# torchmd/torchmd-net

Hardware: AMD Instinct MI355X
Metric: molecules/sec (64-atom molecules) TensorNet E+F (higher is better)
Workload: dtype f32; 1 GPU; BASELINE configs[1]: TensorNet F=128 L=2 K=32 rc=5.0, S-mol64 256 molecules x 64 atoms per GPU, energies + forces, random-init weights (seed 0); atoms_per_gpu=16384, pairs_per_gpu=193709, directed_edges_per_gpu=403802, parallelism=molecule-sharded x1, RCCL all-reduce of energies, rank_step=eager: tmdnet_build_graph (pair-count read-back) + tmdnet_energy_forces

## Files before the change

### torchmd-net_amd/csrc/tn_api.hip

```cpp
#include <hip/hip_runtime.h>

#include <algorithm>
#include <cmath>
#include <cstdio>
#include <cstdlib>
#include <cstring>
#include <map>
#include <unordered_map>
#include <string>
#include <vector>

#include "tn_chain.h"
#include "tn_heads.h"
#include "tn_model.h"
#include "tn_tlin9.h"
#include "tn_small.h"
#include "tn_interp.h"
#include "tn_virial.h"

using namespace tn;

static const char* kCatNames[CAT_COUNT] = {"graph", "gemm_edge", "gemm_node", "message", "pair_bwd", "embed_scatter", "elementwise", "edge_table"};

int fail(tmdnet_model* m, int code, const std::string& msg) {
  if (m) m->err = msg;
  return code;
}
thread_local tmdnet_model* g_cur = nullptr;
thread_local int g_gemm_cat = CAT_GEMM_NODE;
thread_local const int* g_mdev = nullptr;
thread_local int g_madd = 0;
thread_local const uint16_t* g_wsb_debug = nullptr;

void gemm(hipStream_t s, const float* A, int64_t lda, const float* W, int64_t ldw, const float* bias, float* C, int64_t ldc, int M,
          int N, int K, int flags, float* pre, int64_t ldpre, const float* aux, int64_t ldaux,
          const float* rowscale) {
  GemmArgs a{};
  a.A = A;
  a.W[0] = W;
  a.C = C;
  a.bias[0] = bias;
  a.pre = pre;
  a.aux = aux;
  a.rowscale = rowscale;
  a.lda = lda;
// ... 183 lines not shown
  g.counts = c.take<int>(8);
  g.mstart = c.take<int>(B);
  g.mend = c.take<int>(B);
  g.nlow = c.take<int>(N);
  g.ntot = c.take<int>(N);
  g.rowptr = c.take<int>(N + 1);
  g.pairptr = c.take<int>(N + 1);
  g.col = c.take<int>(ecap);
  g.epair = c.take<int>(ecap);
  g.esign = c.take<float>(ecap);
  g.pair_i = c.take<int>(pcap);
  g.pair_j = c.take<int>(pcap);
  g.pd = c.take<float>(pcap + 1);
  g.pdelta = c.take<float>(pcap * 3);
  g.prhat = c.take<float>(pcap * 3);
  g.ecap = ecap;
  g.pcap = pcap;
  g.perm = c.take<int>(N);
  g.iota = c.take<int>(N);
  g.cell_key = c.take<int>(N);
  g.cell_key_sorted = c.take<int>(N);
  g.cell_start = c.take<int>(8 * N + 2);
  g.pos_s = c.take<float>(3 * N);
  g.z_s = c.take<int64_t>(N);
  g.boxd = c.take<float>(12);
  g.cgrid = c.take<int>(4);
  g.bat_s = c.take<int>(N);
  g.bat_c = c.take<int64_t>(N);
  g.z_c = c.take<int64_t>(N);
  g.tix = c.take<int>(N);
  g.tz = c.take<int>(64);
  g.sort_tmp_bytes = cell_sort_temp_bytes(N);
  g.sort_tmp = c.take<char>((int64_t)g.sort_tmp_bytes);
  if (total) *total = c.off;
  return g;
}

namespace {
bool cell_applicable(const tmdnet_model* m, int64_t n_atoms, int64_t n_mol, int box_mode) {
  const int* n = m->cell_n;
  if (n_mol < 1 || box_mode == 2 || n_atoms < 1) return false;
  if (n[0] < 0) return true;
  if (n[0] < 1 || n[1] < 1 || n[2] < 1) return false;
  return (int64_t)n[0] * n[1] * n[2] <= 8 * n_atoms;
}
void set_cell(Graph& g, const tmdnet_model* m, bool on, int64_t n_mol = 1) {
  g.use_cell = on ? (n_mol > 1 ? 2 : 1) : 0;
  const bool explicit_grid = m->cell_n[0] > 0;
  g.ncx = explicit_grid ? m->cell_n[0] : 0;
  g.ncy = explicit_grid ? m->cell_n[1] : 0;
  g.ncz = explicit_grid ? m->cell_n[2] : 0;
}

}
int rb_ntp(const tmdnet_model* m, int64_t n_atoms, int64_t n_pairs) {
  if (!m->rb_fwd || m->et || m->train || n_pairs < 0 || n_atoms < m->rb_min_atoms) return 0;
  return embed_rb_ntp(m->last_nt);
}
namespace {

FwdBuffers carve_fwd(void* ws, const tmdnet_hparams& hp, int64_t N, int64_t B, int64_t P, bool bwd, size_t* total, int ntp = 0,
                     int lean = 0) {
  Carver c(ws);
  FwdBuffers b{};
  const int64_t F = hp.hidden_channels, K = hp.num_rbf, L = hp.num_layers, Z = hp.max_z, H = hp.head_hidden;
  const int64_t P1 = P + 1, N9 = N * 9 * F;
// ... 782 lines not shown
  for (const auto& j : m->image_jobs) {
    if (j.fm) launch_split_weight_fm(m->dev + j.src_off, j.n, j.k, m->dev_sb + j.dst_off, s);
    else launch_split_weight_tiles(m->dev + j.src_off, j.n, j.k, m->dev_sb + j.dst_off, s);
  }
  const int F = m->hp.hidden_channels;
  launch_ztables(m->P.emb, m->P.emb2_waT, m->P.emb2_wbT, m->P.emb2_b, m->hp.max_z, F, const_cast<float*>(m->P.Utab),
                 const_cast<float*>(m->P.Vtab), s);
  m->tabs_pending = true;
  if (m->rb_fwd)
    launch_embed_rb_images(m->P.Wdp, m->P.bdp, F, m->hp.num_rbf, m->rb_img, m->rb_img + embed_rb_image_elems(F, m->hp.num_rbf, false), s);
  HIP_TRY(m, hipGetLastError());
  return TMDNET_OK;
}

int tmdnet_set_option(tmdnet_model* m, const char* name, double value) {
  if (!m || !name) return TMDNET_ERR_INVALID;
  const std::string n(name);
  if (n == "edge_table_min_pairs") {
    m->tab_min_pairs = value < 0 ? 0 : (int64_t)value;
    return TMDNET_OK;
  }
  if (n == "embed_rb_min_atoms") {
    m->rb_min_atoms = value < 0 ? 0 : (int64_t)value;
    return TMDNET_OK;
  }
  if (n == "chain_min_atoms") {
    m->chain_min_atoms = value < 0 ? 0 : (value > 9e18 ? INT64_MAX : (int64_t)value);
    return TMDNET_OK;
  }
  if (n == "chain_mask") {
    m->chain_mask = (int)value & 7;
    return TMDNET_OK;
  }
  if (n == "pair_rows_bf16") {
    if (!m->et) return fail(m, TMDNET_ERR_INVALID, "pair_rows_bf16 applies to the Equivariant Transformer handle only");
    m->pair_bf16 = value == 2.0 ? 2 : (value != 0.0 ? 1 : 0);
    return TMDNET_OK;
  }
  if (n == "recompute_pair_rows") {
    if (m->et || m->tn2) return fail(m, TMDNET_ERR_INVALID, "recompute_pair_rows applies to the TensorNet handle only");
    m->recompute_rows = value != 0.0;
    return TMDNET_OK;
  }
  return fail(m, TMDNET_ERR_INVALID, "unknown option: " + n);
}

int tmdnet_get_info(const tmdnet_model* m, const char* name, double* value) {
  if (!m || !name || !value) return TMDNET_ERR_INVALID;
  const std::string n(name);
  if (m->tabs_pending && n.rfind("edge_table_", 0) == 0 && n != "edge_table_min_pairs")
    if (const int rc = ensure_radial_tables(const_cast<tmdnet_model*>(m), nullptr)) return rc;
  if (n == "edge_table_T") *value = m->tabs.ok ? m->tabs.T : 0;
  else if (n == "edge_table_err_value") *value = m->tabs.err_value;
  else if (n == "edge_table_err_slope") *value = m->tabs.err_slope;
  else if (n == "edge_table_min_pairs") *value = (double)m->tab_min_pairs;
  else if (n == "pair_rows_bf16") *value = (double)m->pair_bf16;
  else if (n == "embed_rb_min_atoms") *value = (double)m->rb_min_atoms;
  else if (n == "chain_min_atoms") *value = (double)m->chain_min_atoms;
  else if (n == "chain_mask") *value = (double)m->chain_mask;
  else if (n == "chain_last") *value = (double)m->chain_last;
  else if (n == "recompute_pair_rows") *value = m->recompute_rows ? 1.0 : 0.0;
  else if (n == "embed_rb") *value = m->rb_fwd ? 1.0 : 0.0;
  else if (n == "species_last_build") *value = (double)m->last_nt;
  else if (n == "halo_active_first") *value = (double)m->halo_active[0];
  else if (n == "halo_active_rows") *value = (double)m->halo_active[1];
  else if (n == "message_route_last") *value = (double)m->msg_route_last[0];
  else if (n == "message_adjoint_route_last") *value = (double)m->msg_route_last[1];
  else return TMDNET_ERR_INVALID;
  return TMDNET_OK;
}

int tmdnet_set_cell_grid(tmdnet_model* m, int32_t ncx, int32_t ncy, int32_t ncz) {
  if (!m) return TMDNET_ERR_INVALID;
  if (ncx < 0 || ncy < 0 || ncz < 0) ncx = ncy = ncz = -1;
  m->cell_n[0] = ncx;
  m->cell_n[1] = ncy;
  m->cell_n[2] = ncz;
  return TMDNET_OK;
}

int tmdnet_graph_workspace_bytes(const tmdnet_model* m, int64_t n_atoms, int64_t n_mol, size_t* bytes) {
  if (!m || !bytes || n_atoms < 0 || n_mol < 0) return TMDNET_ERR_INVALID;
  const int64_t ecap = (int64_t)m->hp.max_num_neighbors * n_atoms;
  carve_graph(nullptr, n_atoms, n_mol, ecap, bytes);
  return TMDNET_OK;
}

int tmdnet_build_graph(tmdnet_model* m, void* stream, void* graph_ws, size_t graph_ws_bytes, int64_t n_atoms, int64_t n_mol,
                       const float* pos, const int64_t* batch, const int64_t* z, const float* box, int32_t box_mode,
                       int64_t counts_host[8]) {
  if (!m || !graph_ws || !counts_host || n_atoms < 0 || n_mol < 0) return TMDNET_ERR_INVALID;
  if (n_atoms >= (int64_t)1 << 30) return fail(m, TMDNET_ERR_INVALID, "n_atoms too large for 32-bit indices");
  hipStream_t s = reinterpret_cast<hipStream_t>(stream);
  const int64_t ecap = (int64_t)m->hp.max_num_neighbors * n_atoms;
  size_t need = 0;
  Graph g = carve_graph(graph_ws, n_atoms, n_mol, ecap, &need);
  if (need > graph_ws_bytes) return fail(m, TMDNET_ERR_WORKSPACE, "graph workspace too small");
  if (box_mode != 0 && !box) return fail(m, TMDNET_ERR_INVALID, "box_mode != 0 needs a box");
  const bool cell = cell_applicable(m, n_atoms, n_mol, box_mode);
  set_cell(g, m, cell, n_mol);
  if (cell && m->halo_fn && m->atom_w && !m->et && !m->tn2) g.ghost_w = m->atom_w;
  m->graph_no_ghost_pairs = g.ghost_w != nullptr;
  m->graph_is_cell = cell;
  m->graph_cell_multi = cell && n_mol > 1;
  m->graph_has_z = z != nullptr;
  m->g_pos = pos;
  m->g_box = box;
  m->g_box_mode = box_mode;
  CurScope cur_(m);
  {
    ProfScope ps_(s, CAT_GRAPH, 0.0, (double)n_atoms * 20);
    if (cell) {
      launch_fill(reinterpret_cast<float*>(g.counts), 0.f, 8, s);
      launch_cell_phase1(g, pos, batch, box_mode == 1 ? box : nullptr, (int)n_atoms, m->hp.cutoff_lower, m->hp.cutoff_upper, true, s,
                         (int)n_mol);
      launch_scan_counts(g, (int)n_atoms, s);
    } else {
      launch_graph_build_phase1(g, pos, batch, box, box_mode, (int)n_atoms, (int)n_mol, m->hp.cutoff_lower, m->hp.cutoff_upper,
                                true, s);
    }
    if (z) launch_prepare_z(g, z, cell ? g.perm : nullptr, (int)n_atoms, m->hp.max_z, s);
    if (z && m->rb_fwd && n_atoms >= m->rb_min_atoms) launch_type_map(g, (int)n_atoms, m->hp.max_z, s);
  }
  int counts[8] = {0, 0, 0, 0, 0, 0, 0, 0};
  HIP_TRY(m, hipMemcpyAsync(counts, g.counts, sizeof(counts), hipMemcpyDeviceToHost, s));
  HIP_TRY(m, hipStreamSynchronize(s));
  for (int k = 0; k < 8; ++k) counts_host[k] = counts[k];
  m->last_nt = (z && m->rb_fwd && n_atoms >= m->rb_min_atoms) ? counts[6] : 0;
  m->lastE = counts[1];
  remember_graph(m, graph_ws);
  if (counts[5])
    return fail(m, TMDNET_ERR_INVALID, "batch index out of range: every entry must be in [0, " + std::to_string(n_mol) + ")");
  if (counts[4])
    return fail(m, TMDNET_ERR_INVALID, "atomic number out of range: every z must be in [0, max_z = " + std::to_string(m->hp.max_z) + ")");
  if (counts[2])
    return fail(m, TMDNET_ERR_OVERFLOW, "Found num_pairs > max_num_pairs, please increase max_num_pairs (found " +
                                            std::to_string(counts[1]) + " edges, capacity " + std::to_string(ecap) + ")");
  m->lastE = counts[1];
  {
    ProfScope ps_(s, CAT_GRAPH, 0.0, (double)counts[1] * 12 + (double)counts[0] * 40);
    if (cell) {
      launch_cell_phase2(g, (int)n_atoms, m->hp.cutoff_lower, m->hp.cutoff_upper, true, s);
      launch_nbr_link_wave(g, (int)n_atoms, s);
    } else {
      launch_graph_build_phase2(g, pos, batch, box, box_mode, (int)n_atoms, (int)n_mol, m->hp.cutoff_lower, m->hp.cutoff_upper, true,
                                s);
    }
  }
  HIP_TRY(m, hipGetLastError());
  return TMDNET_OK;
}

int tmdnet_build_graph_static(tmdnet_model* m, void* stream, void* graph_ws, size_t graph_ws_bytes, int64_t n_atoms, int64_t n_mol,
                              const float* pos, const int64_t* batch, const int64_t* z, const float* box, int32_t box_mode) {
  if (!m || !graph_ws || n_atoms < 0 || n_mol < 0) return TMDNET_ERR_INVALID;
  hipStream_t s = reinterpret_cast<hipStream_t>(stream);
  const int64_t ecap = (int64_t)m->hp.max_num_neighbors * n_atoms;
  size_t need = 0;
  Graph g = carve_graph(graph_ws, n_atoms, n_mol, ecap, &need);
  if (need > graph_ws_bytes) return fail(m, TMDNET_ERR_WORKSPACE, "graph workspace too small");
  if (box_mode != 0 && !box) return fail(m, TMDNET_ERR_INVALID, "box_mode != 0 needs a box");
  const bool cell = cell_applicable(m, n_atoms, n_mol, box_mode);
  set_cell(g, m, cell, n_mol);
  m->graph_no_ghost_pairs = false;
  m->graph_is_cell = cell;
  m->graph_cell_multi = cell && n_mol > 1;
  m->graph_has_z = z != nullptr;
  m->g_pos = pos;
  m->g_box = box;
  m->g_box_mode = box_mode;
  CurScope cur_(m);
  {
    ProfScope ps_(s, CAT_GRAPH, 0.0, (double)n_atoms * 20);
    if (cell) {
      launch_fill(reinterpret_cast<float*>(g.counts), 0.f, 8, s);
      launch_cell_phase1(g, pos, batch, box_mode == 1 ? box : nullptr, (int)n_atoms, m->hp.cutoff_lower, m->hp.cutoff_upper, true, s,
// ... 826 lines not shown
  }
  m->prof.on = false;
  m->prof.recs.clear();
  m->prof.used = 0;
  return TMDNET_OK;
}

int tmdnet_profile_end_records(tmdnet_model* m, void* stream, int64_t cap, int32_t* cat, double* ms, double* flops, double* bytes,
                               char* labels, int64_t* n_out) {
  if (!m || !cat || !ms || !flops || !bytes || !n_out || cap < 0) return TMDNET_ERR_INVALID;
  HIP_TRY(m, hipStreamSynchronize(reinterpret_cast<hipStream_t>(stream)));
  int64_t n = 0;
  for (const ProfRec& r : m->prof.recs) {
    if (n >= cap) break;
    float t = 0.f;
    HIP_TRY(m, hipEventElapsedTime(&t, r.a, r.b));
    cat[n] = r.cat;
    ms[n] = t;
    flops[n] = r.flops;
    bytes[n] = r.bytes;
    if (labels) std::memcpy(labels + 64 * n, r.label, 64);
    ++n;
  }
  *n_out = (int64_t)m->prof.recs.size();
  m->prof.on = false;
  m->prof.recs.clear();
  m->prof.used = 0;
  return TMDNET_OK;
}

int tmdnet_profile_num_categories(void) { return CAT_COUNT; }
const char* tmdnet_profile_category_name(int idx) { return idx >= 0 && idx < CAT_COUNT ? kCatNames[idx] : nullptr; }

int tmdnet_debug_tensor(tmdnet_model* m, void* stream, const char* name, float* out, int64_t numel) {
  if (m && m->et) return et_debug_tensor(m, reinterpret_cast<hipStream_t>(stream), name, out, numel);
  if (!m || !name || !out || !m->has_last) return TMDNET_ERR_STATE;
  hipStream_t s = reinterpret_cast<hipStream_t>(stream);
  const int64_t F = m->hp.hidden_channels, K = m->hp.num_rbf, N = m->lastN, P1 = m->lastP + 1;
  const FwdBuffers& b = m->last;
  const float* src = nullptr;
  int64_t n = 0;
  std::string nm(name);
  if (nm == "X_embed") { src = b.X[0]; n = N * 9 * F; }
  else if (nm.rfind("X_layer", 0) == 0) {
    int l = std::atoi(nm.c_str() + 7);
    if (l < 0 || l >= m->hp.num_layers) return TMDNET_ERR_INVALID;
    src = b.X[l + 1]; n = N * 9 * F;
  }
  else if (nm.rfind("Pn", 0) == 0 || nm.rfind("Mi", 0) == 0 || (nm.rfind("D", 0) == 0 && nm.size() == 2)) {
    const int l = std::atoi(nm.c_str() + (nm[0] == 'D' ? 1 : 2));
    if (l < 0 || l >= m->hp.num_layers) return TMDNET_ERR_INVALID;
    src = nm[0] == 'P' ? b.Pn[l] : (nm[0] == 'M' ? b.Mi[l] : b.D[l]);
    n = N * 9 * F;
  }
  else if (nm == "x") { src = b.x; n = N * F; }
  else if (nm == "phi") { src = b.phi; n = P1 * K; }
  else if (nm == "Q") { src = b.Q; n = P1 * 3 * F; }
  else if (nm == "u0") { src = b.u0; n = N * 9 * F; }
  else if (nm == "G_embed") { src = b.G; n = N * 9 * F; }
  else if (nm == "charges" && m->tn2) { src = m->tn2_last_chg; n = N * (int64_t)(m->hp.num_layers + 1) * m->tn2->hp.q_dim; }
  else return fail(m, TMDNET_ERR_INVALID, "unknown debug tensor");
  if (!src || numel != n) return fail(m, TMDNET_ERR_INVALID, "debug tensor size mismatch: expected " + std::to_string(n));
  HIP_TRY(m, hipMemcpyAsync(out, src, sizeof(float) * n, hipMemcpyDeviceToDevice, s));
  return TMDNET_OK;
}

int tmdnet_debug_gemm_dual(void* stream, const float* A, const float* A2, const float* W, const float* bias, float* C, float* C2,
// ... 207 lines not shown
```

### torchmd-net_amd/csrc/tn_graph_wave.hip

```cpp
#include <cstdlib>

#include "tn_common.h"
#include "tn_kernels.h"

namespace tn {

static inline int cdivw(int64_t a, int64_t b) { return (int)((a + b - 1) / b); }

__device__ __forceinline__ float pair_d2(const float* __restrict__ pos, int hi, int lo, const float* __restrict__ box, float& dx,
                                         float& dy, float& dz) {
  return pair_geometry(pos, hi, lo, box, dx, dy, dz);
}

template <bool FILL>
__device__ __forceinline__ void nbr_wave_row(const Graph& g, const float* __restrict__ pos, const int64_t* __restrict__ batch,
                                             const float* __restrict__ box, int box_mode, int N, int B, float lo2, float up2, int loop,
                                             int i, int lane) {
  int64_t b = batch[i];
  int j0 = 0, j1 = N;
  if (b < 0 || b >= B) {
    b = 0;
    j1 = 0;
  } else if (!g.counts[3]) {
    j0 = g.mstart[b];
    j1 = g.mend[b];
  }
  const float* bx = box_mode == 0 ? nullptr : (box_mode == 1 ? box : box + b * 9);
  const int P = FILL ? g.counts[0] : 0;
  int e = FILL ? g.rowptr[i] : 0, p = FILL ? g.pairptr[i] : 0;
  int nl = 0, nt = 0;
  const unsigned long long lt = lane == 0 ? 0ull : (~0ull >> (64 - lane));
  for (int base = j0; base < j1; base += 64) {
    const int j = base + lane;
    bool hit = false, self = false;
    float dx = 0.f, dy = 0.f, dz = 0.f, d2 = 0.f;
// ... 40 lines not shown
  }
  if (!FILL && lane == 0) {
    g.nlow[i] = nl;
    g.ntot[i] = nt;
  }
  if (FILL && i == 0 && lane == 0) g.pd[P] = 0.f;
}

template <bool FILL>
__global__ __launch_bounds__(256) void k_nbr_wave(Graph g, const float* __restrict__ pos, const int64_t* __restrict__ batch,
                                                  const float* __restrict__ box, int box_mode, int N, int B, float lo2, float up2,
                                                  int loop) {
  const int i = blockIdx.x * 4 + (threadIdx.x >> 6);
  const int lane = threadIdx.x & 63;
  if (i >= N) return;
  if (FILL && g.counts[2]) return;
  nbr_wave_row<FILL>(g, pos, batch, box, box_mode, N, B, lo2, up2, loop, i, lane);
}

__device__ __forceinline__ void nbr_link_row(const Graph& g, int i, int lane) {
  const int e0 = g.rowptr[i], e1 = g.rowptr[i + 1];
  for (int e = e0 + lane; e < e1; e += 64) {
    const int j = g.col[e];
    if (j <= i) continue;
    int lo = g.rowptr[j], hi = lo + g.nlow[j] - 1;
    const int base = lo;
    while (lo < hi) {
      const int mid = (lo + hi) >> 1;
      if (g.col[mid] < i) lo = mid + 1; else hi = mid;
    }
    g.epair[e] = g.pairptr[j] + (lo - base);
  }
}
__global__ __launch_bounds__(256) void k_nbr_link_wave(Graph g, int N) {
  const int i = blockIdx.x * 4 + (threadIdx.x >> 6);
  const int lane = threadIdx.x & 63;
  if (i >= N || g.counts[2]) return;
  nbr_link_row(g, i, lane);
}

constexpr int GS_MAX_ATOMS = 256;
constexpr int GS_ECAP = 16384;
__global__ __launch_bounds__(1024) void k_graph_small(Graph g, const float* __restrict__ pos, const int64_t* __restrict__ batch,
                                                      const float* __restrict__ box, int box_mode, int N, int B, float lo2, float up2,
                                                      int loop, const int64_t* __restrict__ z, int max_z) {
  __shared__ int s_mstart[GS_MAX_ATOMS], s_mend[GS_MAX_ATOMS], s_nlow[GS_MAX_ATOMS], s_ntot[GS_MAX_ATOMS];
  __shared__ int s_rowptr[GS_MAX_ATOMS + 1], s_pairptr[GS_MAX_ATOMS + 1], s_counts[8], c_low[4], c_tot[4];
  __shared__ float s_pos[3 * GS_MAX_ATOMS];
  __shared__ int64_t s_batch[GS_MAX_ATOMS];
  __shared__ int s_col[GS_ECAP];
  const bool col_lds = g.ecap <= GS_ECAP;
  const int tid = threadIdx.x, lane = tid & 63, wave = tid >> 6;
  const bool mol_lds = B <= GS_MAX_ATOMS;
  Graph gl = g;
  gl.nlow = s_nlow;
  gl.ntot = s_ntot;
  gl.rowptr = s_rowptr;
  gl.pairptr = s_pairptr;
  gl.counts = s_counts;
  if (mol_lds) {
    gl.mstart = s_mstart;
    gl.mend = s_mend;
  }
  if (col_lds) gl.col = s_col;
  for (int k = tid; k < 3 * N; k += 1024) s_pos[k] = pos[k];
  if (tid < N) s_batch[tid] = batch[tid];
  for (int i = tid; i < B; i += 1024) gl.mstart[i] = gl.mend[i] = 0;
  if (tid < 8) s_counts[tid] = 0;
  __syncthreads();
  if (tid < N) {
// ... 66 lines not shown
  if (!s_counts[2]) {
    for (int i = wave; i < N; i += 16) nbr_wave_row<true>(gl, s_pos, s_batch, box, box_mode, N, B, lo2, up2, loop, i, lane);
    __syncthreads();
    for (int i = wave; i < N; i += 16) nbr_link_row(gl, i, lane);
    if (col_lds) {
      __syncthreads();
      const int E = s_counts[1];
      for (int e = tid; e < E; e += 1024) g.col[e] = s_col[e];
    }
  }
  if (tid <= N) {
    g.rowptr[tid] = s_rowptr[tid];
    g.pairptr[tid] = s_pairptr[tid];
  }
  if (tid < N) {
    g.nlow[tid] = s_nlow[tid];
    g.ntot[tid] = s_ntot[tid];
  }
  if (mol_lds && tid < B) {
    g.mstart[tid] = s_mstart[tid];
    g.mend[tid] = s_mend[tid];
  }
  if (tid < 8) g.counts[tid] = s_counts[tid];
}
bool graph_small_ok(int N) {
  static const bool off = getenv("TMDNET_NO_GRAPH_SMALL") != nullptr;
  return !off && N > 0 && N <= GS_MAX_ATOMS;
}
void launch_graph_small(const Graph& g, const float* pos, const int64_t* batch, const float* box, int box_mode, int N, int B, float lo,
                        float up, bool loop, const int64_t* z, int max_z, hipStream_t s) {
  hipLaunchKernelGGL(k_graph_small, dim3(1), dim3(1024), 0, s, g, pos, batch, box, box_mode, N, B, lo * lo, up * up, (int)loop, z, max_z);
}

void launch_nbr_count_wave(const Graph& g, const float* pos, const int64_t* batch, const float* box, int box_mode, int N, int B,
                           float lo, float up, bool loop, hipStream_t s) {
  hipLaunchKernelGGL(k_nbr_wave<false>, dim3(cdivw(N, 4)), dim3(256), 0, s, g, pos, batch, box, box_mode, N, B, lo * lo, up * up,
                     (int)loop);
}
void launch_nbr_fill_link_wave(const Graph& g, const float* pos, const int64_t* batch, const float* box, int box_mode, int N, int B,
                               float lo, float up, bool loop, hipStream_t s) {
  hipLaunchKernelGGL(k_nbr_wave<true>, dim3(cdivw(N, 4)), dim3(256), 0, s, g, pos, batch, box, box_mode, N, B, lo * lo, up * up,
                     (int)loop);
  hipLaunchKernelGGL(k_nbr_link_wave, dim3(cdivw(N, 4)), dim3(256), 0, s, g, N);
}
void launch_nbr_link_wave(const Graph& g, int N, hipStream_t s) {
  hipLaunchKernelGGL(k_nbr_link_wave, dim3(cdivw(N, 4)), dim3(256), 0, s, g, N);
}

}
```

### torchmd-net_amd/csrc/tn_kernels.h

```cpp
#pragma once
#include <hip/hip_runtime.h>
#include <stdint.h>

namespace tn {

struct Graph {
  int* mstart;
  int* mend;
  int* nlow;
  int* ntot;
  int* rowptr;
  int* pairptr;
  int* col;
  int* epair;
  float* esign;
  int* pair_i;
  int* pair_j;
  float* pd;
  float* pdelta;
  float* prhat;
  int* counts;
  int* tix;
  int* tz;
  int64_t ecap, pcap;
  int* perm;
  int* iota;
  int* cell_key;
  int* cell_key_sorted;
  int* cell_start;
  float* pos_s;
  int64_t* z_s;
  float* boxd;
  int* cgrid;
  int* bat_s;
  int64_t* bat_c;
  int64_t* z_c;
  void* sort_tmp;
  size_t sort_tmp_bytes;
  int ncx, ncy, ncz;
  int use_cell;
  const float* ghost_w;
  int max_z;
  int small_mols;
};

struct RadialParams {
  const float* means;
  const float* betas;
  int K;
  float lo, up;
};

void launch_graph_build_phase1(const Graph& g, const float* pos, const int64_t* batch, const float* box, int box_mode, int N,
                               int B, float lo, float up, bool loop, hipStream_t s);
void launch_graph_build_phase2(const Graph& g, const float* pos, const int64_t* batch, const float* box, int box_mode, int N,
                               int B, float lo, float up, bool loop, hipStream_t s);
void launch_export_pairs(const Graph& g, int N, bool include_transpose, bool loop, int64_t max_pairs, const int* perm,
                         int64_t* neighbors, float* deltas, float* distances, int* num_pairs, hipStream_t s);

void launch_neighbor_grad(const int64_t* nb, const float* deltas, const float* dist, const float* g_delta, const float* g_dist,
                          int64_t M, int N, float* out, hipStream_t s);

void launch_radial(const Graph& g, int P, RadialParams rp, float* phi, float* dphi, float* C, float* dC, hipStream_t s);

void launch_ztables(const float* emb, const float* WaT, const float* WbT, const float* b2, int Z, int F, float* Utab, float* Vtab,
                    hipStream_t s);
void launch_embed_scatter(const Graph& g, int N, int F, const int64_t* z, const float* Utab, const float* Vtab, const float* Q,
                          const float* C, float* u0, float* s0n, hipStream_t s);
void launch_layernorm_fwd(const float* x, const float* w, const float* b, int rows, int R, float* y, float* xhat, float* rstd,
                          hipStream_t s);
void launch_layernorm_bwd(const float* g, const float* xhat, const float* rstd, const float* w, int rows, int R, float* gx,
                          hipStream_t s);
void launch_norm_x(const float* X, float* Xh, int N, int F, hipStream_t s);
struct PairRowTable;
enum MsgRoute {
  MSG_NONE = 0,
// ... 51 lines not shown

void launch_head_bwd(const float* ao, const float* O2, int N, int H, float std, float* g_ao, hipStream_t s);
void launch_readout_bwd(const float* X, const float* g_feat, int N, int F, float* G, hipStream_t s);
void launch_update_bwd(const float* G, const float* D, const float* q, const int64_t* batch, int N, int F, float* gD,
                       hipStream_t s);
void launch_message_bwd_node(const float* gCh, const float* Pn, const float* Mi, const float* q, const int64_t* batch, int o3, int N,
                             int F, float* gMi, float* gPn, hipStream_t s);
void launch_norm_bwd(const float* X, const float* gXh_lin, int N, int F, float* G, hipStream_t s);
void launch_norm_bwd_update_bwd(const float* X, const float* gXh_lin, int N, int F, float* G, const float* Dn, const float* q,
                                const int64_t* batch, float* gD, hipStream_t s);
void launch_norm_bwd_gate_bwd(const float* X, const float* gXh_lin, int N, int F, float* G, const float* UX, const float* gates,
                              const float* a2, float* gUX, float* g_a2, hipStream_t s);
void launch_lnbwd_readout_bwd(const float* g, const float* xhat, const float* rstd, const float* w, int N, int F, const float* X,
                              float* G, hipStream_t s);
void launch_head_mol_sum(const Graph& g, const float* ao, const float* O2, const float* bO2, int N, int B, int H, float std,
                         const float* atomref, const int64_t* z, const int64_t* batch, float mean, float* energy, hipStream_t s,
                         float* g_ao = nullptr, const float* atom_w = nullptr, const int* perm = nullptr);
void launch_embed_gate_bwd(const float* G, const float* UX, const float* gates, const float* a2, int N, int F, float* gUX, float* g_a2,
                           hipStream_t s);
void launch_owned_range(const float* aw, const int* perm, int N, int* out, hipStream_t s);
void launch_embed_bwd_atom(const float* g_u0_lin, const float* u0, const float* g_s0n, int N, int F, float* gA, hipStream_t s);
void launch_force_gather(const Graph& g, int N, const float* g_delta, const int* perm, float* forces, hipStream_t s,
                         const float* direct = nullptr);
void launch_fill(float* p, float v, int64_t n, hipStream_t s);
void launch_kappa(const float* q, const int64_t* batch, int N, int B, float* kap, hipStream_t s);

void launch_nbr_count_wave(const Graph& g, const float* pos, const int64_t* batch, const float* box, int box_mode, int N, int B,
                           float lo, float up, bool loop, hipStream_t s);
void launch_nbr_fill_link_wave(const Graph& g, const float* pos, const int64_t* batch, const float* box, int box_mode, int N, int B,
                               float lo, float up, bool loop, hipStream_t s);

void launch_nbr_link_wave(const Graph& g, int N, hipStream_t s);
bool graph_small_ok(int N);
void launch_graph_small(const Graph& g, const float* pos, const int64_t* batch, const float* box, int box_mode, int N, int B, float lo,
                        float up, bool loop, const int64_t* z, int max_z, hipStream_t s);
void launch_scan_counts(const Graph& g, int N, hipStream_t s);

size_t cell_sort_temp_bytes(int64_t n);
void launch_cell_phase1(const Graph& g, const float* pos, const int64_t* batch, const float* box, int N, float lo, float up, bool loop,
                        hipStream_t s, int B = 0);
void launch_cell_phase2(const Graph& g, int N, float lo, float up, bool loop, hipStream_t s);
void launch_permute_z(const Graph& g, const int64_t* z, int N, hipStream_t s);
void launch_prepare_z(const Graph& g, const int64_t* z, const int* perm, int N, int max_z, hipStream_t s);

void launch_pair_gd(const Graph& g, int Pcap, int F, const float* gMi, const float* Pn, const float* dw, float* gd, hipStream_t s);
void launch_embed_pair_gd(const Graph& g, int Pcap, int F, const int64_t* z, const float* Utab, const float* Vtab, const float* Q,
                          const float* dQ, const float* C, const float* dC, const float* gA, float* gd, float* g_rhat, hipStream_t s,
                          float* g_delta = nullptr, const float* slots = nullptr, int n_slots = 0, int64_t slot_stride = 0);
void launch_geom_gd(const Graph& g, int Pcap, const float* gd, const float* g_rhat, float* g_delta, hipStream_t s,
                    const float* slots = nullptr, int n_slots = 0, int64_t slot_stride = 0);

void launch_radial_f64(int rows, double lo, double up, int T, bool mid, const float* means, const float* betas, int K, double* dist,
                       double* phi, double* dphi, double* C, double* dC, hipStream_t s);
void launch_dense_f64(const double* A, const double* A2, int lda, const float* W, const float* bias, int M, int N, int K, int kind,
                      const double* rs, const double* rs2, double* C, double* C2, int ldc, hipStream_t s);
void launch_table_pack(const double* f, const double* sl, int T, int R, double h, float* tab, hipStream_t s);
void launch_pair_buckets(const Graph& g, int Pcap, float lo, float up, int T, float* C, float* dC, int* hist, unsigned* keys_s,
                         int* vals_s, hipStream_t s);
bool edge_interp_direct(int Pcap);
void launch_edge_interp(const Graph& g, int Pcap, float lo, float up, int T, int R, int ntab, const float* const* tabs,
                        float* const* outs, float* const* douts, const unsigned* keys_s, const int* vals_s, hipStream_t s, float* C,
                        float* dC, int out_bf16 = 0);
void launch_type_map(const Graph& g, int N, int max_z, hipStream_t s);
bool embed_rb_shape_ok(int F, int K);
int embed_rb_ntp(int nt);
int64_t embed_rb_moment_elems(int64_t N, int ntp, int K);
// ... 22 lines not shown
```

### torchmd-net_amd/csrc/tn_model.h

```cpp
#pragma once
#include <hip/hip_runtime.h>

#include <cstdio>
#include <cstring>
#include <map>
#include <string>
#include <unordered_map>
#include <vector>

#include "../../include/tmdnet_amd.h"
#include "tn_gemm.h"
#include "tn_kernels.h"
#include "tn_train.h"

using namespace tn;


struct LayerP {
  const float *M1, *b1, *M2, *b2, *M3, *b3;
  const float *M2T, *M3T;
  const float* V[6];
  const float* VT[6];
  const uint16_t* M_sb[3];
};
// ... 116 lines not shown
  float *part = nullptr, *wT = nullptr, *forces = nullptr;
  float* at(const std::string& k) const { return grads + off.at(k); }
};

struct tmdnet_model {
  bool recompute_rows = false;
  const float* atom_w = nullptr;
  int (*halo_fn)(void*, int32_t, float*, int64_t, int64_t, const int32_t*, void*) = nullptr;
  void* halo_user = nullptr;
  int* halo_rng = nullptr;
  bool graph_no_ghost_pairs = false;
  int halo_active[2] = {0, 0};
  int msg_route_last[2] = {0, 0};
  tmdnet_hparams hp;
  int head_kind = 0;
  TrainCtx* train = nullptr;
  float* virial_out = nullptr;
  void* virial_ws = nullptr;
  std::vector<std::pair<std::string, int64_t>> train_entries;
  hipStream_t side = nullptr;
  hipEvent_t ev_fork = nullptr;
  std::vector<hipEvent_t> ev_join;
  EtModel* et = nullptr;
  Tn2Model* tn2 = nullptr;
  const float* g_pos = nullptr;
  const float* g_box = nullptr;
  int g_box_mode = 0;
  Profiler prof;
  int64_t lastE = 0;
  int cell_n[3] = {0, 0, 0};
  bool graph_is_cell = false;
  bool graph_cell_multi = false;
  bool graph_has_z = false;
  struct GraphRecord { bool is_cell, cell_multi, has_z; int nt; int64_t lastE; bool no_ghost_pairs; };
  std::unordered_map<const void*, GraphRecord> graph_rec;
  std::vector<ParamSpec> specs;
  std::map<std::string, std::vector<float>> host;
  float* dev = nullptr;
  size_t dev_cap = 0, dev_sb_cap = 0, rb_cap = 0;
  uint16_t* dev_sb = nullptr;
  std::unordered_map<const float*, const uint16_t*> sb_of;
  std::unordered_map<const float*, const uint16_t*> fm_of;
  struct ImageJob { size_t src_off; int64_t n, k; size_t dst_off; int fm; };
  std::vector<ImageJob> image_jobs;
  size_t packed_elems = 0;
  int32_t* upd_tid = nullptr;
  int32_t* upd_ofs = nullptr;
  const float** upd_ptrs = nullptr;
  bool upd_ready = false;
  DevParams P;
  EdgeTables tabs;
  uint16_t* rb_img = nullptr;
  const uint16_t *rb_fwd = nullptr, *rb_rev = nullptr;
  int last_nt = 0;
  int64_t rb_min_atoms = 1024;
  int64_t chain_min_atoms = 4096;
  int chain_mask = 7;
  int chain_last = 0;
  int pair_bf16 = 0;
  bool tabs_pending = false;
  int64_t tab_min_pairs = 1;
  bool finalized = false;
  std::string err;
  FwdBuffers last{};
  int64_t lastN = 0, lastP = 0;
  bool has_last = false;
// ... 101 lines not shown
```

Baseline: 108,700 molecules/s.

## Add fused block-batched neighbor graph build for sorted small-molecule batches

Adds a new non-cell graph-build route: one kernel per 64-row block counts neighbours using per-row molecule runs found with wave ballots, and folds in z clamping and species bitmaps. A single-block kernel then scans the per-block totals and builds the species rank table. A fill kernel writes columns into shared memory and links edges in place for blocks whose molecules are fully contained, falling back to the global link kernel for open blocks. This replaces the separate prepare_z, type_map, scan and link launches and targets per-launch and global-memory costs of graph construction, at the cost of more complex code and a retry path with an extra host sync when batches are unsorted. It also adds a graph debug-tensor readout.

Result: faster. 110,500 molecules/s (median of 6 runs) (+1.6%).

```diff
diff --git a/torchmd-net_amd/csrc/tn_api.hip b/torchmd-net_amd/csrc/tn_api.hip
--- a/torchmd-net_amd/csrc/tn_api.hip
+++ b/torchmd-net_amd/csrc/tn_api.hip
@@ -11,6 +11,7 @@
 #include <vector>
 
 #include "tn_chain.h"
+#include "tn_graph_batch_math.h"
 #include "tn_heads.h"
 #include "tn_model.h"
 #include "tn_tlin9.h"
@@ -260,6 +261,16 @@
   g.tz = c.take<int>(64);
   g.sort_tmp_bytes = cell_sort_temp_bytes(N);
   g.sort_tmp = c.take<char>((int64_t)g.sort_tmp_bytes);
+  const int64_t nblk = gb_blocks(N) <= GB_MAX_BLOCKS ? gb_blocks(N) : 0;
+  g.gb_low = c.take<int>(nblk);
+  g.gb_tot = c.take<int>(nblk);
+  g.gb_flag = c.take<int>(nblk);
+  g.gb_closed = c.take<int>(nblk);
+  g.gb_blow = c.take<int>(nblk);
+  g.gb_btot = c.take<int>(nblk);
+  g.gb_bits = c.take<unsigned>(nblk * GB_ZWORDS);
+  g.gb_rank = c.take<int>(nblk ? GB_MAX_Z : 0);
+  if (!nblk) g.gb_low = nullptr;
   if (total) *total = c.off;
   return g;
 }
@@ -1108,6 +1119,10 @@
     m->chain_mask = (int)value & 7;
     return TMDNET_OK;
   }
+  if (n == "graph_batch") {
+    m->graph_batch = value != 0.0;
+    return TMDNET_OK;
+  }
   if (n == "pair_rows_bf16") {
     if (!m->et) return fail(m, TMDNET_ERR_INVALID, "pair_rows_bf16 applies to the Equivariant Transformer handle only");
     m->pair_bf16 = value == 2.0 ? 2 : (value != 0.0 ? 1 : 0);
@@ -1134,6 +1149,8 @@
   else if (n == "embed_rb_min_atoms") *value = (double)m->rb_min_atoms;
   else if (n == "chain_min_atoms") *value = (double)m->chain_min_atoms;
   else if (n == "chain_mask") *value = (double)m->chain_mask;
+  else if (n == "graph_batch") *value = m->graph_batch ? 1.0 : 0.0;
+  else if (n == "graph_route_last") *value = (double)m->graph_route_last;
   else if (n == "chain_last") *value = (double)m->chain_last;
   else if (n == "recompute_pair_rows") *value = m->recompute_rows ? 1.0 : 0.0;
   else if (n == "embed_rb") *value = m->rb_fwd ? 1.0 : 0.0;
@@ -1184,25 +1201,42 @@
   m->g_box = box;
   m->g_box_mode = box_mode;
   CurScope cur_(m);
-  {
-    ProfScope ps_(s, CAT_GRAPH, 0.0, (double)n_atoms * 20);
-    if (cell) {
-      launch_fill(reinterpret_cast<float*>(g.counts), 0.f, 8, s);
-      launch_cell_phase1(g, pos, batch, box_mode == 1 ? box : nullptr, (int)n_atoms, m->hp.cutoff_lower, m->hp.cutoff_upper, true, s,
-                         (int)n_mol);
-      launch_scan_counts(g, (int)n_atoms, s);
-    } else {
-      launch_graph_build_phase1(g, pos, batch, box, box_mode, (int)n_atoms, (int)n_mol, m->hp.cutoff_lower, m->hp.cutoff_upper,
-                                true, s);
-    }
-    if (z) launch_prepare_z(g, z, cell ? g.perm : nullptr, (int)n_atoms, m->hp.max_z, s);
-    if (z && m->rb_fwd && n_atoms >= m->rb_min_atoms) launch_type_map(g, (int)n_atoms, m->hp.max_z, s);
-  }
+  const bool want_types = z && m->rb_fwd && n_atoms >= m->rb_min_atoms;
+  bool batch_route = !cell && m->graph_batch && graph_batch_ok(g, n_atoms, n_mol, z ? m->hp.max_z : 0);
+  m->graph_route_last = cell ? 1 : (batch_route ? 2 : 0);
   int counts[8] = {0, 0, 0, 0, 0, 0, 0, 0};
-  HIP_TRY(m, hipMemcpyAsync(counts, g.counts, sizeof(counts), hipMemcpyDeviceToHost, s));
-  HIP_TRY(m, hipStreamSynchronize(s));
-  for (int k = 0; k < 8; ++k) counts_host[k] = counts[k];
-  m->last_nt = (z && m->rb_fwd && n_atoms >= m->rb_min_atoms) ? counts[6] : 0;
+  for (;;) {
+    {
+      ProfScope ps_(s, CAT_GRAPH, 0.0, (double)n_atoms * 20);
+      if (cell) {
+        launch_fill(reinterpret_cast<float*>(g.counts), 0.f, 8, s);
+        launch_cell_phase1(g, pos, batch, box_mode == 1 ? box : nullptr, (int)n_atoms, m->hp.cutoff_lower, m->hp.cutoff_upper, true, s,
+                           (int)n_mol);
+        launch_scan_counts(g, (int)n_atoms, s);
+      } else if (batch_route) {
+        launch_graph_batch_phase1(g, pos, batch, box, box_mode, (int)n_atoms, (int)n_mol, m->hp.cutoff_lower, m->hp.cutoff_upper, true,
+                                  z, m->hp.max_z, want_types, s);
+      } else {
+        launch_graph_build_phase1(g, pos, batch, box, box_mode, (int)n_atoms, (int)n_mol, m->hp.cutoff_lower, m->hp.cutoff_upper,
+                                  true, s);
+      }
+      if (!batch_route) {
+        if (z) launch_prepare_z(g, z, cell ? g.perm : nullptr, (int)n_atoms, m->hp.max_z, s);
+        if (want_types) launch_type_map(g, (int)n_atoms, m->hp.max_z, s);
+      }
+    }
+    HIP_TRY(m, hipMemcpyAsync(counts, g.counts, sizeof(counts), hipMemcpyDeviceToHost, s));
+    HIP_TRY(m, hipStreamSynchronize(s));
+    if (!(batch_route && (counts[7] & GB_R_FALLBACK))) break;
+    batch_route = false;
+    m->graph_route_last = 3;
+  }
+  for (int k = 0; k < 7; ++k) counts_host[k] = counts[k];
+  counts_host[7] = 0;
+  m->dbg_graph_ws = graph_ws;
+  m->dbg_graph_dims[0] = n_atoms, m->dbg_graph_dims[1] = n_mol, m->dbg_graph_dims[2] = counts[0], m->dbg_graph_dims[3] = counts[1];
+  m->dbg_graph_types = want_types;
+  m->last_nt = want_types ? counts[6] : 0;
   m->lastE = counts[1];
   remember_graph(m, graph_ws);
   if (counts[5])
@@ -1218,6 +1252,9 @@
     if (cell) {
       launch_cell_phase2(g, (int)n_atoms, m->hp.cutoff_lower, m->hp.cutoff_upper, true, s);
       launch_nbr_link_wave(g, (int)n_atoms, s);
+    } else if (batch_route) {
+      launch_graph_batch_phase2(g, pos, batch, box, box_mode, (int)n_atoms, (int)n_mol, m->hp.cutoff_lower, m->hp.cutoff_upper, true,
+                                want_types, (counts[7] & GB_R_OPEN) != 0, s);
     } else {
       launch_graph_build_phase2(g, pos, batch, box, box_mode, (int)n_atoms, (int)n_mol, m->hp.cutoff_lower, m->hp.cutoff_upper, true,
                                 s);
@@ -2110,7 +2147,39 @@
 int tmdnet_profile_num_categories(void) { return CAT_COUNT; }
 const char* tmdnet_profile_category_name(int idx) { return idx >= 0 && idx < CAT_COUNT ? kCatNames[idx] : nullptr; }
 
+static int debug_graph_field(tmdnet_model* m, hipStream_t s, const std::string& f, float* out, int64_t numel) {
+  if (!m->dbg_graph_ws) return fail(m, TMDNET_ERR_STATE, "no dynamic graph build yet");
+  const int64_t N = m->dbg_graph_dims[0], B = m->dbg_graph_dims[1], P = m->dbg_graph_dims[2], E = m->dbg_graph_dims[3];
+  const Graph g = carve_graph(m->dbg_graph_ws, N, B, (int64_t)m->hp.max_num_neighbors * N, nullptr);
+  const void* src = nullptr;
+  int64_t n = 0;
+  if (f == "counts") { src = g.counts; n = 8; }
+  else if (f == "mstart") { src = g.mstart; n = B; }
+  else if (f == "mend") { src = g.mend; n = B; }
+  else if (f == "nlow") { src = g.nlow; n = N; }
+  else if (f == "ntot") { src = g.ntot; n = N; }
+  else if (f == "rowptr") { src = g.rowptr; n = N + 1; }
+  else if (f == "pairptr") { src = g.pairptr; n = N + 1; }
+  else if (f == "col") { src = g.col; n = E; }
+  else if (f == "epair") { src = g.epair; n = E; }
+  else if (f == "esign") { src = g.esign; n = E; }
+  else if (f == "pair_i") { src = g.pair_i; n = P; }
+  else if (f == "pair_j") { src = g.pair_j; n = P; }
+  else if (f == "pd") { src = g.pd; n = P + 1; }
+  else if (f == "pdelta") { src = g.pdelta; n = 3 * P; }
+  else if (f == "prhat") { src = g.prhat; n = 3 * P; }
+  else if (f == "z_c" && m->graph_has_z) { src = g.z_c; n = 2 * N; }
+  else if (f == "tix" && m->dbg_graph_types) { src = g.tix; n = N; }
+  else if (f == "tz" && m->dbg_graph_types) { src = g.tz; n = 64; }
+  else return fail(m, TMDNET_ERR_INVALID, "unknown debug tensor");
+  if (numel != n) return fail(m, TMDNET_ERR_INVALID, "debug tensor size mismatch: expected " + std::to_string(n));
+  if (n > 0) HIP_TRY(m, hipMemcpyAsync(out, src, sizeof(float) * n, hipMemcpyDeviceToDevice, s));
+  return TMDNET_OK;
+}
+
 int tmdnet_debug_tensor(tmdnet_model* m, void* stream, const char* name, float* out, int64_t numel) {
+  if (m && name && out && std::strncmp(name, "graph_", 6) == 0)
+    return debug_graph_field(m, reinterpret_cast<hipStream_t>(stream), std::string(name + 6), out, numel);
   if (m && m->et) return et_debug_tensor(m, reinterpret_cast<hipStream_t>(stream), name, out, numel);
   if (!m || !name || !out || !m->has_last) return TMDNET_ERR_STATE;
   hipStream_t s = reinterpret_cast<hipStream_t>(stream);
diff --git a/torchmd-net_amd/csrc/tn_graph_batch_math.h b/torchmd-net_amd/csrc/tn_graph_batch_math.h
--- /dev/null
+++ b/torchmd-net_amd/csrc/tn_graph_batch_math.h
@@ -0,0 +1,69 @@
+#pragma once
+#include <stdint.h>
+
+#if defined(__HIPCC__) || defined(__CUDACC__)
+#define TN_GB_HD __host__ __device__ inline
+#else
+#define TN_GB_HD inline
+#endif
+
+namespace tn {
+
+constexpr int GB_ROWS = 64;
+constexpr int GB_MAX_BLOCKS = 1024;
+constexpr int GB_CHUNK = 16;
+constexpr int GB_ZWORDS = 64;
+constexpr int GB_MAX_Z = GB_ZWORDS * 32;
+constexpr int GB_RUN_CAP = 4096;
+
+enum : int { GB_F_BATCH_RANGE = 1, GB_F_Z_RANGE = 2, GB_F_UNSORTED = 4, GB_F_RUN_CAP = 8 };
+enum : int { GB_R_RAN = 1, GB_R_FALLBACK = 2, GB_R_OPEN = 4 };
+
+TN_GB_HD int gb_blocks(int64_t N) { return (int)((N + GB_ROWS - 1) / GB_ROWS); }
+
+TN_GB_HD void gb_gap_before(int64_t bp, int64_t b, int& k0, int& k1) {
+  k0 = (int)(bp + 1);
+  k1 = bp < b ? (int)b : k0;
+}
+TN_GB_HD void gb_gap_after(int64_t b, int B, int& k0, int& k1) {
+  k0 = (int)(b + 1);
+  k1 = B > k0 ? B : k0;
+}
+
+TN_GB_HD bool gb_row_closed(int j0, int j1, int blk, int N) {
+  const int r0 = blk * GB_ROWS, r1 = r0 + GB_ROWS < N ? r0 + GB_ROWS : N;
+  return j1 <= j0 || (j0 >= r0 && j1 <= r1);
+}
+
+TN_GB_HD int gb_chunk_sum(const int* v, int c, int n) {
+  int s = 0;
+  for (int k = c * GB_CHUNK; k < (c + 1) * GB_CHUNK && k < n; ++k) s += v[k];
+  return s;
+}
+TN_GB_HD void gb_chunk_scan(const int* v, int c, int n, int base, int* out) {
+  for (int k = c * GB_CHUNK; k < (c + 1) * GB_CHUNK && k < n; ++k) {
+    out[k] = base;
+    base += v[k];
+  }
+}
+
+TN_GB_HD int gb_popc(uint32_t x) {
+  int n = 0;
+  for (; x; x &= x - 1) ++n;
+  return n;
+}
+TN_GB_HD void gb_rank_word(uint32_t word, int w, int base, int max_z, int* rank, int* tz) {
+  for (int bit = 0; bit < 32; ++bit) {
+    const int z = w * 32 + bit;
+    if (z >= max_z) return;
+    if (word >> bit & 1u) {
+      rank[z] = base;
+      if (base < 64) tz[base] = z;
+      ++base;
+    } else {
+      rank[z] = -1;
+    }
+  }
+}
+
+}
diff --git a/torchmd-net_amd/csrc/tn_graph_wave.hip b/torchmd-net_amd/csrc/tn_graph_wave.hip
--- a/torchmd-net_amd/csrc/tn_graph_wave.hip
+++ b/torchmd-net_amd/csrc/tn_graph_wave.hip
@@ -1,6 +1,7 @@
 #include <cstdlib>
 
 #include "tn_common.h"
+#include "tn_graph_batch_math.h"
 #include "tn_kernels.h"
 
 namespace tn {
@@ -107,10 +108,11 @@
     g.epair[e] = g.pairptr[j] + (lo - base);
   }
 }
-__global__ __launch_bounds__(256) void k_nbr_link_wave(Graph g, int N) {
+__global__ __launch_bounds__(256) void k_nbr_link_wave(Graph g, int N, const int* __restrict__ closed) {
   const int i = blockIdx.x * 4 + (threadIdx.x >> 6);
   const int lane = threadIdx.x & 63;
   if (i >= N || g.counts[2]) return;
+  if (closed && closed[i / GB_ROWS]) return;
   nbr_link_row(g, i, lane);
 }
 
@@ -243,6 +245,302 @@
   hipLaunchKernelGGL(k_graph_small, dim3(1), dim3(1024), 0, s, g, pos, batch, box, box_mode, N, B, lo * lo, up * up, (int)loop, z, max_z);
 }
 
+constexpr int GBF_ECAP = 8192;
+
+template <class T>
+__device__ __forceinline__ T* rebase(T* slot0, int64_t index0) {
+  return reinterpret_cast<T*>(reinterpret_cast<uintptr_t>(slot0) - (uintptr_t)index0 * sizeof(T));
+}
+
+__device__ __forceinline__ bool batch_run(const int64_t* __restrict__ batch, int N, int i, int64_t b, int lane, int& j0, int& j1) {
+  bool ok = true;
+  int s = i, e = i + 1;
+  for (int step = 0;; ++step) {
+    if (step == GB_RUN_CAP / 64) {
+      ok = false;
+      break;
+    }
+    const int j = s - 1 - lane;
+    const unsigned long long m = __ballot(j >= 0 && batch[j] == b);
+    const int run = m == ~0ull ? 64 : __builtin_ctzll(~m);
+    s -= run;
+    if (run < 64) break;
+  }
+  for (int step = 0;; ++step) {
+    if (step == GB_RUN_CAP / 64) {
+      ok = false;
+      break;
+    }
+    const int j = e + lane;
+    const unsigned long long m = __ballot(j < N && batch[j] == b);
+    const int run = m == ~0ull ? 64 : __builtin_ctzll(~m);
+    e += run;
+    if (run < 64) break;
+  }
+  j0 = s;
+  j1 = e;
+  return ok;
+}
+
+__global__ __launch_bounds__(1024) void k_graph_batch_count(Graph g, const float* __restrict__ pos, const int64_t* __restrict__ batch,
+                                                            const float* __restrict__ box, int box_mode, int N, int B, float lo2,
+                                                            float up2, int loop, const int64_t* __restrict__ z, int max_z,
+                                                            int want_types) {
+  __shared__ int s_j0[GB_ROWS], s_j1[GB_ROWS], s_nl[GB_ROWS], s_nt[GB_ROWS], s_counts[8], s_flag, s_open;
+  __shared__ unsigned s_bits[GB_ZWORDS];
+  const int tid = threadIdx.x, lane = tid & 63, wave = tid >> 6;
+  const int blk = blockIdx.x, r0 = blk * GB_ROWS;
+  if (tid < GB_ZWORDS) s_bits[tid] = 0u;
+  if (tid < GB_ROWS) s_nl[tid] = s_nt[tid] = 0;
+  if (tid < 8) s_counts[tid] = 0;
+  if (tid == 0) s_flag = s_open = 0;
+  __syncthreads();
+  if (z && tid < GB_ROWS && r0 + tid < N) {
+    int64_t v = z[r0 + tid];
+    if (v < 0 || v >= max_z) {
+      atomicOr(&s_flag, (int)GB_F_Z_RANGE);
+      v = v < 0 ? 0 : max_z - 1;
+    }
+    g.z_c[r0 + tid] = v;
+    if (want_types) atomicOr(&s_bits[(int)v >> 5], 1u << ((int)v & 31));
+  }
+  int64_t b_prev = -1;
+  int j0 = 0, j1 = 0;
+  for (int r = 0; r < 4; ++r) {
+    const int li = wave * 4 + r, i = r0 + li;
+    if (i >= N) break;
+    const int64_t b = batch[i];
+    int flags = 0;
+    if (b < 0 || b >= B) {
+      flags = GB_F_BATCH_RANGE;
+      j0 = j1 = 0;
+      b_prev = -1;
+    } else {
+      const int64_t bp = i > 0 ? batch[i - 1] : -1, bn = i < N - 1 ? batch[i + 1] : -1;
+      if (bp > b) flags |= GB_F_UNSORTED;
+      if (!(b == b_prev && i < j1)) {
+        if (!batch_run(batch, N, i, b, lane, j0, j1)) flags |= GB_F_RUN_CAP;
+        b_prev = b;
+      }
+      if (i == 0 || bp != b) {
+        if (lane == 0) g.mstart[b] = i;
+        if (bp >= -1) {
+          int k0, k1;
+          gb_gap_before(bp, b, k0, k1);
+          for (int k = k0 + lane; k < k1; k += 64) g.mstart[k] = g.mend[k] = 0;
+        }
+      }
+      if (i == N - 1 || bn != b) {
+        if (lane == 0) g.mend[b] = i + 1;
+        if (i == N - 1) {
+          int k0, k1;
+          gb_gap_after(b, B, k0, k1);
+          for (int k = k0 + lane; k < k1; k += 64) g.mstart[k] = g.mend[k] = 0;
+        }
+      }
+    }
+    if (lane == 0) {
+      s_j0[li] = j0;
+      s_j1[li] = j1;
+      if (flags) atomicOr(&s_flag, flags);
+      if (!gb_row_closed(j0, j1, blk, N)) s_open = 1;
+    }
+    __builtin_amdgcn_fence(__ATOMIC_RELEASE, "wavefront");
+    __builtin_amdgcn_wave_barrier();
+    __builtin_amdgcn_fence(__ATOMIC_ACQUIRE, "wavefront");
+    if (!flags || flags == GB_F_UNSORTED) {
+      Graph gl = g;
+      gl.counts = s_counts;
+      gl.mstart = rebase(&s_j0[li], b);
+      gl.mend = rebase(&s_j1[li], b);
+      gl.nlow = rebase(s_nl, r0);
+      gl.ntot = rebase(s_nt, r0);
+      nbr_wave_row<false>(gl, pos, batch, box, box_mode, N, B, lo2, up2, loop, i, lane);
+    }
+  }
+  __syncthreads();
+  if (wave == 0) {
+    const int i = r0 + lane;
+    const int nl = s_nl[lane], nt = s_nt[lane];
+    int a = nl, b = nt;
+#pragma unroll
+    for (int off = 1; off < 64; off <<= 1) {
+      const int ta = __shfl_up(a, off, 64), tb = __shfl_up(b, off, 64);
+      if (lane >= off) {
+        a += ta;
+        b += tb;
+      }
+    }
+    if (i < N) {
+      g.nlow[i] = nl;
+      g.ntot[i] = nt;
+      g.pairptr[i] = a - nl;
+      g.rowptr[i] = b - nt;
+    }
+    if (lane == 63) {
+      g.gb_low[blk] = a;
+      g.gb_tot[blk] = b;
+      g.gb_flag[blk] = s_flag;
+      g.gb_closed[blk] = s_open ? 0 : 1;
+    }
+    g.gb_bits[blk * GB_ZWORDS + lane] = s_bits[lane];
+  }
+}
+
+__global__ __launch_bounds__(1024) void k_graph_batch_finalise(Graph g, int N, int nblk, int have_z, int max_z, int want_types) {
+  __shared__ int s_low[GB_MAX_BLOCKS], s_tot[GB_MAX_BLOCKS], s_blow[GB_MAX_BLOCKS], s_btot[GB_MAX_BLOCKS];
+  __shared__ int s_rank[GB_MAX_Z], s_tz[64], s_flag, s_open, s_sum[3];
+  __shared__ unsigned s_bits[GB_ZWORDS];
+  const int tid = threadIdx.x, lane = tid & 63, wave = tid >> 6;
+  if (tid < GB_ZWORDS) {
+    s_bits[tid] = 0u;
+    s_tz[tid] = 0;
+  }
+  if (tid == 0) s_flag = s_open = 0;
+  __syncthreads();
+  if (tid < nblk) {
+    const int tot = g.gb_tot[tid];
+    s_low[tid] = g.gb_low[tid];
+    s_tot[tid] = tot;
+    const int f = g.gb_flag[tid];
+    if (f) atomicOr(&s_flag, f);
+    const int closed = g.gb_closed[tid] && tot <= GBF_ECAP;
+    g.gb_closed[tid] = closed;
+    if (!closed) s_open = 1;
+  }
+  if (want_types) {
+    unsigned w = 0u;
+    for (int k = wave; k < nblk; k += 16 * 8) {
+      unsigned t[8];
+#pragma unroll
+      for (int u = 0; u < 8; ++u) t[u] = k + 16 * u < nblk ? g.gb_bits[(k + 16 * u) * GB_ZWORDS + lane] : 0u;
+#pragma unroll
+      for (int u = 0; u < 8; ++u) w |= t[u];
+    }
+    if (w) atomicOr(&s_bits[lane], w);
+  }
+  __syncthreads();
+  if (wave == 0) {
+    const int a = gb_chunk_sum(s_low, lane, nblk), b = gb_chunk_sum(s_tot, lane, nblk);
+    int ia = a, ib = b;
+#pragma unroll
+    for (int off = 1; off < 64; off <<= 1) {
+      const int ta = __shfl_up(ia, off, 64), tb = __shfl_up(ib, off, 64);
+      if (lane >= off) {
+        ia += ta;
+        ib += tb;
+      }
+    }
+    gb_chunk_scan(s_low, lane, nblk, ia - a, s_blow);
+    gb_chunk_scan(s_tot, lane, nblk, ib - b, s_btot);
+    if (lane == 63) {
+      s_sum[0] = ia;
+      s_sum[1] = ib;
+    }
+  } else if (wave == 1 && want_types) {
+    const unsigned w = s_bits[lane];
+    const int c = gb_popc(w);
+    int ic = c;
+#pragma unroll
+    for (int off = 1; off < 64; off <<= 1) {
+      const int t = __shfl_up(ic, off, 64);
+      if (lane >= off) ic += t;
+    }
+    gb_rank_word(w, lane, ic - c, max_z, s_rank, s_tz);
+    if (lane == 63) s_sum[2] = ic;
+  }
+  __syncthreads();
+  if (tid < nblk) {
+    g.gb_blow[tid] = s_blow[tid];
+    g.gb_btot[tid] = s_btot[tid];
+  }
+  if (want_types) {
+    for (int k = tid; k < max_z; k += 1024) g.gb_rank[k] = s_rank[k];
+    if (tid < 64) g.tz[tid] = s_tz[tid];
+  }
+  if (tid == 0) {
+    const int P = s_sum[0], E = s_sum[1], f = s_flag;
+    const int oob = f & GB_F_BATCH_RANGE ? 1 : 0;
+    g.pairptr[N] = P;
+    g.rowptr[N] = E;
+    g.counts[0] = P;
+    g.counts[1] = E;
+    g.counts[2] = (E > g.ecap || P > g.pcap || oob) ? 1 : 0;
+    g.counts[3] = (oob || (f & GB_F_UNSORTED)) ? 1 : 0;
+    g.counts[4] = (have_z && (f & GB_F_Z_RANGE)) ? 1 : 0;
+    g.counts[5] = oob;
+    g.counts[6] = want_types ? s_sum[2] : 0;
+    g.counts[7] = GB_R_RAN | ((f & (GB_F_BATCH_RANGE | GB_F_UNSORTED | GB_F_RUN_CAP)) ? GB_R_FALLBACK : 0) | (s_open ? GB_R_OPEN : 0);
+  }
+}
+
+__global__ __launch_bounds__(1024) void k_graph_batch_fill(Graph g, const float* __restrict__ pos, const int64_t* __restrict__ batch,
+                                                           const float* __restrict__ box, int box_mode, int N, int B, float lo2,
+                                                           float up2, int loop, int want_types) {
+  __shared__ int s_rowptr[GB_ROWS + 1], s_pairptr[GB_ROWS + 1], s_nl[GB_ROWS], s_counts[8];
+  __shared__ int s_col[GBF_ECAP];
+  const int tid = threadIdx.x, lane = tid & 63, wave = tid >> 6;
+  const int blk = blockIdx.x, r0 = blk * GB_ROWS;
+  const int nrows = N - r0 < GB_ROWS ? N - r0 : GB_ROWS;
+  if (tid < 8) s_counts[tid] = tid == 3 ? 0 : g.counts[tid];
+  const int e_base = g.gb_btot[blk], p_base = g.gb_blow[blk];
+  if (tid < nrows) {
+    const int i = r0 + tid;
+    const int e = g.rowptr[i] + e_base, p = g.pairptr[i] + p_base;
+    s_rowptr[tid] = e;
+    s_pairptr[tid] = p;
+    s_nl[tid] = g.nlow[i];
+    g.rowptr[i] = e;
+    g.pairptr[i] = p;
+    if (want_types) g.tix[i] = g.gb_rank[(int)g.z_c[i]];
+  }
+  if (tid == nrows) {
+    s_rowptr[nrows] = e_base + g.gb_tot[blk];
+    s_pairptr[nrows] = p_base + g.gb_low[blk];
+  }
+  const bool closed = g.gb_closed[blk] != 0;
+  __syncthreads();
+  if (s_counts[2]) return;
+  Graph gl = g;
+  gl.counts = s_counts;
+  gl.rowptr = rebase(s_rowptr, r0);
+  gl.pairptr = rebase(s_pairptr, r0);
+  if (closed) {
+    gl.nlow = rebase(s_nl, r0);
+    gl.col = rebase(s_col, e_base);
+  }
+  for (int r = 0; r < 4; ++r) {
+    const int i = r0 + wave * 4 + r;
+    if (i < N) nbr_wave_row<true>(gl, pos, batch, box, box_mode, N, B, lo2, up2, loop, i, lane);
+  }
+  if (!closed) return;
+  __syncthreads();
+  for (int r = 0; r < 4; ++r) {
+    const int i = r0 + wave * 4 + r;
+    if (i < N) nbr_link_row(gl, i, lane);
+  }
+  const int E = s_rowptr[nrows] - e_base;
+  for (int e = tid; e < E; e += 1024) g.col[e_base + e] = s_col[e];
+}
+
+bool graph_batch_ok(const Graph& g, int64_t N, int64_t B, int max_z) {
+  if (getenv("TMDNET_SCALAR_GRAPH")) return false;
+  return N > 0 && g.small_mols && g.gb_low && gb_blocks(N) <= GB_MAX_BLOCKS && max_z <= GB_MAX_Z && B <= 4 * N + 4096;
+}
+void launch_graph_batch_phase1(const Graph& g, const float* pos, const int64_t* batch, const float* box, int box_mode, int N, int B,
+                               float lo, float up, bool loop, const int64_t* z, int max_z, bool want_types, hipStream_t s) {
+  const int nblk = gb_blocks(N);
+  hipLaunchKernelGGL(k_graph_batch_count, dim3(nblk), dim3(1024), 0, s, g, pos, batch, box, box_mode, N, B, lo * lo, up * up, (int)loop,
+                     z, max_z, (int)(z && want_types));
+  hipLaunchKernelGGL(k_graph_batch_finalise, dim3(1), dim3(1024), 0, s, g, N, nblk, (int)(z != nullptr), max_z, (int)(z && want_types));
+}
+void launch_graph_batch_phase2(const Graph& g, const float* pos, const int64_t* batch, const float* box, int box_mode, int N, int B,
+                               float lo, float up, bool loop, bool want_types, bool some_open, hipStream_t s) {
+  hipLaunchKernelGGL(k_graph_batch_fill, dim3(gb_blocks(N)), dim3(1024), 0, s, g, pos, batch, box, box_mode, N, B, lo * lo, up * up,
+                     (int)loop, (int)want_types);
+  if (some_open) hipLaunchKernelGGL(k_nbr_link_wave, dim3(cdivw(N, 4)), dim3(256), 0, s, g, N, (const int*)g.gb_closed);
+}
+
 void launch_nbr_count_wave(const Graph& g, const float* pos, const int64_t* batch, const float* box, int box_mode, int N, int B,
                            float lo, float up, bool loop, hipStream_t s) {
   hipLaunchKernelGGL(k_nbr_wave<false>, dim3(cdivw(N, 4)), dim3(256), 0, s, g, pos, batch, box, box_mode, N, B, lo * lo, up * up,
@@ -252,10 +550,10 @@
                                float lo, float up, bool loop, hipStream_t s) {
   hipLaunchKernelGGL(k_nbr_wave<true>, dim3(cdivw(N, 4)), dim3(256), 0, s, g, pos, batch, box, box_mode, N, B, lo * lo, up * up,
                      (int)loop);
-  hipLaunchKernelGGL(k_nbr_link_wave, dim3(cdivw(N, 4)), dim3(256), 0, s, g, N);
+  hipLaunchKernelGGL(k_nbr_link_wave, dim3(cdivw(N, 4)), dim3(256), 0, s, g, N, (const int*)nullptr);
 }
 void launch_nbr_link_wave(const Graph& g, int N, hipStream_t s) {
-  hipLaunchKernelGGL(k_nbr_link_wave, dim3(cdivw(N, 4)), dim3(256), 0, s, g, N);
-}
-
-}
+  hipLaunchKernelGGL(k_nbr_link_wave, dim3(cdivw(N, 4)), dim3(256), 0, s, g, N, (const int*)nullptr);
+}
+
+}
diff --git a/torchmd-net_amd/csrc/tn_kernels.h b/torchmd-net_amd/csrc/tn_kernels.h
--- a/torchmd-net_amd/csrc/tn_kernels.h
+++ b/torchmd-net_amd/csrc/tn_kernels.h
@@ -42,6 +42,14 @@
   const float* ghost_w;
   int max_z;
   int small_mols;
+  int* gb_low;
+  int* gb_tot;
+  int* gb_flag;
+  int* gb_closed;
+  int* gb_blow;
+  int* gb_btot;
+  unsigned* gb_bits;
+  int* gb_rank;
 };
 
 struct RadialParams {
@@ -159,6 +167,11 @@
 
 void launch_nbr_link_wave(const Graph& g, int N, hipStream_t s);
 bool graph_small_ok(int N);
+bool graph_batch_ok(const Graph& g, int64_t N, int64_t B, int max_z);
+void launch_graph_batch_phase1(const Graph& g, const float* pos, const int64_t* batch, const float* box, int box_mode, int N, int B,
+                               float lo, float up, bool loop, const int64_t* z, int max_z, bool want_types, hipStream_t s);
+void launch_graph_batch_phase2(const Graph& g, const float* pos, const int64_t* batch, const float* box, int box_mode, int N, int B,
+                               float lo, float up, bool loop, bool want_types, bool some_open, hipStream_t s);
 void launch_graph_small(const Graph& g, const float* pos, const int64_t* batch, const float* box, int box_mode, int N, int B, float lo,
                         float up, bool loop, const int64_t* z, int max_z, hipStream_t s);
 void launch_scan_counts(const Graph& g, int N, hipStream_t s);
diff --git a/torchmd-net_amd/csrc/tn_model.h b/torchmd-net_amd/csrc/tn_model.h
--- a/torchmd-net_amd/csrc/tn_model.h
+++ b/torchmd-net_amd/csrc/tn_model.h
@@ -172,6 +172,11 @@
   bool graph_is_cell = false;
   bool graph_cell_multi = false;
   bool graph_has_z = false;
+  bool graph_batch = true;
+  int graph_route_last = 0;
+  void* dbg_graph_ws = nullptr;
+  int64_t dbg_graph_dims[4] = {0, 0, 0, 0};
+  bool dbg_graph_types = false;
   struct GraphRecord { bool is_cell, cell_multi, has_z; int nt; int64_t lastE; bool no_ghost_pairs; };
   std::unordered_map<const void*, GraphRecord> graph_rec;
   std::vector<ParamSpec> specs;
```
